# prototypefund/your-voice-TTS

Measured on AMD Instinct MI355X. Metric: mel-frames/sec + RTF, Tacotron2 + 60-iter Griffin-Lim, LJSpeech, higher is better.
Workload: dtype f32; 1 GPU; configs[1]: Tacotron2 single sentence, HIP decoder loop + HIP Griffin-Lim 60 iters; sentences_per_gpu=1, L=100, gl_iters=60, model_config=config_tacotron2.json + forward_attn_mask (synthesize.py:86), parallelism=single GPU

## Files before the change

include/tts_hip.h:

```cpp
#ifndef TTS_HIP_H
#define TTS_HIP_H

#include <stdint.h>

#ifdef __cplusplus
extern "C" {
#endif

typedef int tts_status;
#define TTS_OK 0
#define TTS_ERR_INVALID 1
#define TTS_ERR_HIP 2
#define TTS_ERR_UNSUPPORTED 3
#define TTS_ERR_NOMEM 4

typedef struct tts_encoder tts_encoder;
typedef struct tts_decoder tts_decoder;
typedef struct tts_postnet tts_postnet;
typedef struct tts_gl tts_gl;
typedef struct tts_tacotron tts_tacotron;

typedef struct tts_tensor {
    const char* key;
    const float* data;
    int64_t numel;
} tts_tensor;

tts_status tts_encoder_create(const tts_tensor* tensors, int n_tensors, int max_batch, int max_len,
                              void* stream, tts_encoder** out);
void tts_encoder_destroy(tts_encoder* e);
tts_status tts_encoder_run(tts_encoder* e, const int32_t* ids, const int32_t* lens, int B, int Lmax,
                           float* out, void* stream);
tts_status tts_encoder_run_state(tts_encoder* e, const int32_t* ids, const int32_t* lens, int B, int Lmax,
                                 const float* state_in, float* state_out, float* out, void* stream);

tts_status tts_encoder_add_speakers(tts_encoder* e, float* enc, const int32_t* lens, const int32_t* speaker_ids, int B,
                                    int Lmax, void* stream);

tts_status tts_encoder_last_path(tts_encoder* e, int* resident);

typedef struct tts_decoder_config {
    int r;
    int attn_norm;
    int forward_attn;
    int trans_agent;
    int forward_attn_mask;
    int location_attn;
    int windowing;
    int max_batch;
    int max_len;
    int max_steps;
} tts_decoder_config;

tts_status tts_decoder_create(const tts_decoder_config* cfg, const tts_tensor* tensors, int n_tensors,
                              void* stream, tts_decoder** out);
void tts_decoder_destroy(tts_decoder* d);

tts_status tts_decoder_run(tts_decoder* d, const float* enc, const int32_t* lens, int B, int Lmax,
                           int max_steps, int steps_cap, float* mel, float* stop, float* align,
                           int32_t* n_steps, void* stream);

tts_status tts_decoder_run_continue(tts_decoder* d, const float* enc, const int32_t* lens, int B, int Lmax,
                                    int max_steps, int steps_cap, float* mel, float* stop, float* align,
                                    int32_t* n_steps, void* stream);

tts_status tts_decoder_run_teacher(tts_decoder* d, const float* enc, const int32_t* lens, int B, int Lmax,
                                   const float* memories, int64_t mem_ldb, int steps, float* mel, float* stop,
                                   float* align, void* stream);

tts_status tts_decoder_last_timing(tts_decoder* d, float* loop_ms, int* steps_run);

tts_status tts_decoder_last_path(tts_decoder* d, int* resident);
// ... 56 lines not shown
                           const int32_t* orig_sr, int target_sr, int B, double* dst, int64_t dst_pitch,
                           int32_t* n_out, void* stream);

tts_status tts_gl_set_mel_basis(tts_gl* g, const double* mel_basis);
tts_status tts_gl_melspectrogram(tts_gl* g, const double* wav, const int32_t* N, int B, int64_t Nmax, float* mel,
                                 int Fmax, void* stream);

tts_status tts_gl_analyze(tts_gl* g, const double* wav, const int32_t* N, int B, int64_t Nmax, float* linear,
                          float* mel, int Fmax, void* stream);

tts_status tts_gl_linear_to_mel(tts_gl* g, const float* linear, const int32_t* F, int B, int Fmax, float* mel,
                                void* stream);

tts_status tts_gl_last_timing(tts_gl* g, float* loop_ms, int* launches);

#define TTS_GL_PATH_UNFUSED 0
#define TTS_GL_PATH_FUSED 1
#define TTS_GL_PATH_PERSISTENT 2
tts_status tts_gl_last_path(tts_gl* g, int* path);

#define TTS_GL_KERNELS 2
tts_status tts_gl_profile(tts_gl* g, int reps, float* kernel_ms, int n_kernels);

typedef struct tts_synth tts_synth;
tts_status tts_synth_create(tts_encoder* e, tts_decoder* d, tts_postnet* p, tts_gl* g, int r, int n_mel, int hop,
                            tts_synth** out);
void tts_synth_destroy(tts_synth* s);
tts_status tts_synth_run(tts_synth* s, const int32_t* ids, const int32_t* lens, int B, int Lmax, int max_steps,
                         int gl_iters, uint64_t seed, double* wav, int64_t wav_cap, int32_t* frames, void* stream);
tts_status tts_synth_run_speakers(tts_synth* s, const int32_t* ids, const int32_t* lens, const int32_t* speaker_ids,
                                  int B, int Lmax, int max_steps, int gl_iters, uint64_t seed, double* wav,
                                  int64_t wav_cap, int32_t* frames, void* stream);
tts_status tts_synth_sync(tts_synth* s);

#define TTS_TACOTRON_MEMORY_SIZE_MAX 16
typedef struct tts_tacotron_config {
    int r;
    int memory_size;
    int attn_norm;
    int forward_attn, trans_agent, forward_attn_mask, location_attn, windowing;
    int gst;
    int num_speakers;
    int max_batch;
    int max_len;
    int max_steps;
} tts_tacotron_config;

tts_status tts_tacotron_create(const tts_tacotron_config* cfg, const tts_tensor* tensors, int n_tensors,
                               void* stream, tts_tacotron** out);
void tts_tacotron_destroy(tts_tacotron* t);

tts_status tts_tacotron_encode(tts_tacotron* t, const int32_t* ids, const int32_t* lens, int B, int Lmax,
                               const int32_t* speaker_ids, const float* style_mel, int style_frames, float* out,
                               void* stream);

tts_status tts_tacotron_decode(tts_tacotron* t, const float* enc, const int32_t* lens, int B, int Lmax,
                               int max_steps, int steps_cap, float* mel, float* stop, float* align,
                               int32_t* n_steps, void* stream);

tts_status tts_tacotron_decode_teacher(tts_tacotron* t, const float* enc, const int32_t* lens, int B, int Lmax,
                                       const float* memories, int64_t mem_ldb, int steps, float* mel,
                                       float* stop, float* align, void* stream);

tts_status tts_tacotron_postnet(tts_tacotron* t, const float* mel, const int32_t* T, int B, int Tmax,
                                float* linear, void* stream);

// ... 70 lines not shown
```

your-voice-tts_amd/_native.py:

```python
from __future__ import annotations

import ctypes
import os
import threading

_HERE = os.path.dirname(os.path.abspath(__file__))
LIB_PATH = os.environ.get("TTS_HIP_LIB", os.path.join(_HERE, "libtts_hip.so"))

TTS_GL_FROM_MEL = 0
TTS_GL_FROM_LINEAR = 1
TTS_LOSS_L1 = 0
TTS_LOSS_MSE = 1
TTS_LOSS_BCE = 2
TTS_OPTIM_CHUNK = 8192
GL_PATHS = {0: "unfused", 1: "fused", 2: "persistent"}
DECODER_STEP_KERNELS = ("prenet2", "att_lstm", "query", "attention", "dec_lstm", "mel_fused")
GL_KERNELS = ("gl_iter", "gl_ola")
TACOTRON_STEP_KERNELS = ("prenet2", "att_gru", "query", "attention", "proj", "dec_gru1", "dec_gru2", "mel",
                         "pre1_stop")

EXPORTS = (
    "tts_encoder_create", "tts_encoder_destroy", "tts_encoder_run", "tts_encoder_run_state", "tts_encoder_last_path",
    "tts_encoder_add_speakers", "tts_synth_run_speakers",
    "tts_decoder_create", "tts_decoder_destroy", "tts_decoder_run", "tts_decoder_run_continue", "tts_decoder_run_teacher",
    "tts_decoder_last_timing", "tts_decoder_last_path", "tts_decoder_resident_limits", "tts_decoder_resident_phases", "tts_decoder_resident_trace",
    "tts_decoder_profile",
    "tts_postnet_create", "tts_postnet_destroy", "tts_postnet_run", "tts_postnet_last_path",
    "tts_gl_create", "tts_gl_destroy", "tts_gl_run", "tts_gl_last_timing", "tts_gl_last_path", "tts_gl_profile",
    "tts_gl_set_mel_basis", "tts_gl_melspectrogram", "tts_gl_set_phase_state", "tts_gl_get_phase_state",
    "tts_gl_draw_phases", "tts_gl_save_pcm16", "tts_gl_analyze", "tts_gl_linear_to_mel",
    "tts_gl_trim_silence", "tts_gl_find_endpoint", "tts_gl_take_segments",
    "tts_gl_set_resample_filter", "tts_gl_resample",
    "tts_synth_create", "tts_synth_destroy", "tts_synth_run", "tts_synth_sync",
    "tts_tacotron_create", "tts_tacotron_destroy", "tts_tacotron_encode", "tts_tacotron_decode",
    "tts_tacotron_decode_teacher",
    "tts_tacotron_postnet", "tts_tacotron_last_timing", "tts_tacotron_last_path", "tts_tacotron_resident_phases",
    "tts_tacotron_profile",
    "tts_loss_create", "tts_loss_destroy", "tts_loss_masked", "tts_loss_bce_logits", "tts_loss_backward",
    "tts_optim_create", "tts_optim_destroy", "tts_optim_set_tensors", "tts_optim_grad_norm", "tts_optim_clip",
    "tts_optim_decay", "tts_optim_adam", "tts_optim_step",
    "tts_last_error", "tts_version",
)


class TensorView(ctypes.Structure):
    _fields_ = [("key", ctypes.c_char_p), ("data", ctypes.c_void_p), ("numel", ctypes.c_int64)]


class DecoderConfig(ctypes.Structure):
    _fields_ = [(n, ctypes.c_int) for n in (
        "r", "attn_norm", "forward_attn", "trans_agent", "forward_attn_mask", "location_attn",
        "windowing", "max_batch", "max_len", "max_steps")]


class TacotronConfig(ctypes.Structure):
    _fields_ = [(n, ctypes.c_int) for n in (
# ... 14 lines not shown
                ("signal_norm", ctypes.c_int), ("symmetric_norm", ctypes.c_int), ("clip_norm", ctypes.c_int)]


_lib = None
_lock = threading.Lock()
P = ctypes.c_void_p
I32P = ctypes.POINTER(ctypes.c_int32)


def _declare(lib):
    vp = ctypes.c_void_p
    lib.tts_encoder_create.argtypes = [ctypes.POINTER(TensorView), ctypes.c_int, ctypes.c_int, ctypes.c_int, vp,
                                       ctypes.POINTER(vp)]
    lib.tts_encoder_destroy.argtypes = [vp]
    lib.tts_encoder_destroy.restype = None
    lib.tts_encoder_run.argtypes = [vp, vp, I32P, ctypes.c_int, ctypes.c_int, vp, vp]
    lib.tts_encoder_add_speakers.argtypes = [vp, vp, I32P, I32P, ctypes.c_int, ctypes.c_int, vp]
    lib.tts_decoder_create.argtypes = [ctypes.POINTER(DecoderConfig), ctypes.POINTER(TensorView), ctypes.c_int, vp,
                                       ctypes.POINTER(vp)]
    lib.tts_decoder_destroy.argtypes = [vp]
    lib.tts_decoder_destroy.restype = None
    lib.tts_decoder_run.argtypes = [vp, vp, I32P, ctypes.c_int, ctypes.c_int, ctypes.c_int, ctypes.c_int, vp, vp, vp,
                                    I32P, vp]
    lib.tts_encoder_run_state.argtypes = [vp, vp, I32P, ctypes.c_int, ctypes.c_int, vp, vp, vp, vp]
    lib.tts_decoder_run_continue.argtypes = lib.tts_decoder_run.argtypes
    lib.tts_decoder_run_teacher.argtypes = [vp, vp, I32P, ctypes.c_int, ctypes.c_int, vp, ctypes.c_int64, ctypes.c_int,
                                            vp, vp, vp, vp]
    lib.tts_decoder_last_timing.argtypes = [vp, ctypes.POINTER(ctypes.c_float), ctypes.POINTER(ctypes.c_int)]
    lib.tts_decoder_last_path.argtypes = [vp, ctypes.POINTER(ctypes.c_int)]
    lib.tts_decoder_resident_limits.argtypes = [vp, ctypes.POINTER(ctypes.c_int), ctypes.POINTER(ctypes.c_int)]
    lib.tts_encoder_last_path.argtypes = [vp, ctypes.POINTER(ctypes.c_int)]
    lib.tts_gl_last_path.argtypes = [vp, ctypes.POINTER(ctypes.c_int)]
    lib.tts_synth_sync.argtypes = [vp]
    lib.tts_decoder_resident_phases.argtypes = [vp, ctypes.POINTER(ctypes.c_float), ctypes.c_int]
    lib.tts_decoder_resident_trace.argtypes = [vp, ctypes.POINTER(ctypes.c_longlong), ctypes.c_int64]
    lib.tts_postnet_create.argtypes = [ctypes.POINTER(TensorView), ctypes.c_int, ctypes.c_int, vp, ctypes.POINTER(vp)]
    lib.tts_postnet_destroy.argtypes = [vp]
    lib.tts_postnet_destroy.restype = None
    lib.tts_postnet_run.argtypes = [vp, vp, I32P, ctypes.c_int, ctypes.c_int, vp, vp]
    lib.tts_postnet_last_path.argtypes = [vp, ctypes.POINTER(ctypes.c_int), ctypes.c_int]
    lib.tts_gl_create.argtypes = [ctypes.POINTER(AudioConfig), vp, vp, ctypes.POINTER(vp)]
    lib.tts_gl_destroy.argtypes = [vp]
    lib.tts_gl_destroy.restype = None
    lib.tts_gl_run.argtypes = [vp, ctypes.c_int, vp, I32P, ctypes.c_int, ctypes.c_int, vp, ctypes.c_uint64,
                               ctypes.c_int, vp, vp]
    lib.tts_gl_set_mel_basis.argtypes = [vp, vp]
    lib.tts_gl_melspectrogram.argtypes = [vp, vp, I32P, ctypes.c_int, ctypes.c_int64, vp, ctypes.c_int, vp]
    lib.tts_gl_analyze.argtypes = [vp, vp, I32P, ctypes.c_int, ctypes.c_int64, vp, vp, ctypes.c_int, vp]
    lib.tts_gl_linear_to_mel.argtypes = [vp, vp, I32P, ctypes.c_int, ctypes.c_int, vp, vp]
    lib.tts_gl_last_timing.argtypes = [vp, ctypes.POINTER(ctypes.c_float), ctypes.POINTER(ctypes.c_int)]
    U32P = ctypes.POINTER(ctypes.c_uint32)
    lib.tts_gl_set_phase_state.argtypes = [vp, U32P, ctypes.c_int]
    lib.tts_gl_get_phase_state.argtypes = [vp, U32P, ctypes.POINTER(ctypes.c_int)]
    lib.tts_gl_draw_phases.argtypes = [vp, I32P, ctypes.c_int, ctypes.c_int, vp, vp]
    lib.tts_gl_save_pcm16.argtypes = [vp, vp, ctypes.c_int64, ctypes.POINTER(ctypes.c_int64), ctypes.c_int, ctypes.c_int,
                                      ctypes.c_double, vp, vp]
    lib.tts_gl_trim_silence.argtypes = [vp, vp, ctypes.c_int64, I32P, ctypes.c_int, ctypes.c_int, ctypes.c_int,
                                        ctypes.c_int, ctypes.c_double, I32P, I32P, vp]
    lib.tts_gl_find_endpoint.argtypes = [vp, vp, ctypes.c_int64, I32P, ctypes.c_int, ctypes.c_int, ctypes.c_int,
                                         ctypes.c_double, I32P, vp]
    lib.tts_gl_take_segments.argtypes = [vp, vp, ctypes.c_int64, I32P, I32P, ctypes.c_int, vp, ctypes.c_int64, vp]
    lib.tts_gl_set_resample_filter.argtypes = [vp, vp, ctypes.c_int, ctypes.c_int]
    lib.tts_gl_resample.argtypes = [vp, vp, ctypes.c_int64, I32P, I32P, ctypes.c_int, ctypes.c_int, vp, ctypes.c_int64,
                                    I32P, vp]
    lib.tts_synth_create.argtypes = [vp, vp, vp, vp, ctypes.c_int, ctypes.c_int, ctypes.c_int, ctypes.POINTER(vp)]
    lib.tts_synth_destroy.argtypes = [vp]
# ... 16 lines not shown
                                                ctypes.c_int, vp, vp, vp, vp]
    lib.tts_tacotron_postnet.argtypes = [vp, vp, I32P, ctypes.c_int, ctypes.c_int, vp, vp]
    lib.tts_tacotron_last_timing.argtypes = [vp, ctypes.POINTER(ctypes.c_float), ctypes.POINTER(ctypes.c_int)]
    lib.tts_tacotron_last_path.argtypes = [vp, ctypes.POINTER(ctypes.c_int)]
    lib.tts_tacotron_resident_phases.argtypes = [vp, FP, ctypes.c_int]
    lib.tts_tacotron_profile.argtypes = [vp, ctypes.c_int, FP, ctypes.c_int]
    DP, I64P = ctypes.POINTER(ctypes.c_double), ctypes.POINTER(ctypes.c_int64)
    lib.tts_loss_create.argtypes = [ctypes.POINTER(vp)]
    lib.tts_loss_destroy.argtypes = [vp]
    lib.tts_loss_destroy.restype = None
    lib.tts_loss_masked.argtypes = [vp, ctypes.c_int, vp, ctypes.c_int64, vp, ctypes.c_int64, I32P, ctypes.c_int,
                                    ctypes.c_int, ctypes.c_int, vp, vp, DP, I64P, DP, vp]
    lib.tts_loss_bce_logits.argtypes = [vp, vp, vp, ctypes.c_int64, vp, vp, DP, DP, vp]
    lib.tts_loss_backward.argtypes = [ctypes.c_int, vp, ctypes.c_int64, vp, ctypes.c_int64, vp, ctypes.c_int,
                                      ctypes.c_int64, ctypes.c_int64, vp, vp, ctypes.c_int64, vp]
    OT, D = ctypes.POINTER(OptimTensor), ctypes.c_double
    lib.tts_optim_create.argtypes = [ctypes.POINTER(vp)]
    lib.tts_optim_destroy.argtypes = [vp]
    lib.tts_optim_destroy.restype = None
    lib.tts_optim_set_tensors.argtypes = [vp, I64P, ctypes.c_int, vp]
    lib.tts_optim_grad_norm.argtypes = [vp, OT, ctypes.c_int, D, vp, vp, DP, DP, vp]
    lib.tts_optim_clip.argtypes = lib.tts_optim_grad_norm.argtypes
    lib.tts_optim_decay.argtypes = [vp, OT, ctypes.c_int, D, D, vp]
    lib.tts_optim_adam.argtypes = [vp, OT, ctypes.c_int, D, D, D, D, vp]
    lib.tts_optim_step.argtypes = [vp, OT, ctypes.c_int, D, D, D, D, D, D, vp, vp, vp]
    lib.tts_last_error.restype = ctypes.c_char_p
    lib.tts_version.restype = ctypes.c_char_p
    for name in EXPORTS:
        fn = getattr(lib, name)
        if name.endswith(("_create", "_run", "_timing", "_profile", "_encode", "_decode", "_postnet", "_state",
                          "_continue", "_basis", "_melspectrogram", "_path", "_sync", "_phases", "_teacher",
                          "_phase_state", "_pcm16", "_limits", "_analyze", "_to_mel", "_silence", "_endpoint",
                          "_segments", "_masked", "_logits", "_filter", "_resample", "_tensors", "_grad_norm",
                          "_clip", "_decay", "_adam", "_step", "_backward")):
            fn.restype = ctypes.c_int


def load_library(path: str = LIB_PATH):
    global _lib
    with _lock:
        if _lib is None:
            import torch
            if not os.path.exists(path):
                raise RuntimeError(f"libtts_hip.so not found at {path}: build it with "
                                   f"`make -C your-voice-tts_amd/csrc` (no CPU fallback exists)")
            lib = ctypes.CDLL(path)
            _declare(lib)
            _lib = lib
    return _lib


def lib():
    import torch
    if not torch.cuda.is_available():
        raise RuntimeError("no GPU visible: the MI355X synthesis path has no CPU fallback")
    return load_library()


def check(status: int, what: str):
    if status != 0:
        msg = load_library().tts_last_error().decode(errors="replace")
        if "attention norm" in msg:
            raise RuntimeError("Unknown value for attention norm type")
        raise RuntimeError(f"{what} failed (status {status}): {msg}")


def stream_handle(stream=None):
# ... 23 lines not shown
```

your-voice-tts_amd/csrc/encoder_api.hip:

```cpp
#include <algorithm>
#include <map>
#include <string>

#include "conv1d.h"
#include "encoder_resident.h"
#include "host_util.h"
#include "resident.h"
#include "sgemm.h"

using namespace tts;

namespace {
constexpr int EDIM = 512;
constexpr int EH = 256;
constexpr int EG = 4 * EH;
}

struct tts_encoder {
    int num_chars = 0, Bcap = 0, Lcap = 0;
    hipStream_t stream = nullptr;
    hipEvent_t ev_in = nullptr, ev_out = nullptr;
    DeviceAllocs dev;
    float* emb = nullptr;
    float* spk = nullptr;
    int nspk = 0;
    float *Wc[3] = {}, *sc[3] = {}, *sh[3] = {};
    float *Wp = nullptr, *bp = nullptr;
    float *Wcf[3] = {}, *Wpf = nullptr;
    float* Wcf16[3] = {};
    float* Whh = nullptr;
    int *ids = nullptr, *T = nullptr;
    float *act0 = nullptr, *act1 = nullptr, *xi = nullptr, *h = nullptr, *c = nullptr, *out = nullptr;
    float* part = nullptr;
    std::map<std::pair<int, int>, hipGraphExec_t> graphs;
    bool resident = false;
    float4* rw = nullptr;
    unsigned long long* rgran = nullptr;
    long long rtmo = 0;
    unsigned rsalt = 0;
    bool rgran_clear = false;
    unsigned rsalt_pending = 0;
    bool pending_batch = false;
    int* host_status = nullptr;
    bool pipeline = false;
    bool status_pending = false;
    bool defer_status = false;
    bool lens_staged = false;
    bool skip_resident_once = false;
    int res_timeouts = 0;
    std::map<int, hipGraphExec_t> rgraphs;
    float* whh_raw = nullptr;
    unsigned long long* bgran = nullptr;
    unsigned bsalt = 0;
    bool bgran_clear = false;
    std::map<std::pair<int, int>, hipGraphExec_t> bgraphs;
    int last_resident = 0;
};

namespace {

__global__ void zero_rows_past_len_kernel(float* out, int Lmax, const int* T) {
    const int t = blockIdx.x, b = blockIdx.y;
    if (t < T[b]) return;
    reinterpret_cast<float4*>(out + ((size_t)b * Lmax + t) * EDIM)[threadIdx.x] = float4{0.f, 0.f, 0.f, 0.f};
}

tts_status enqueue_encoder(tts_encoder* e, int B, int Lmax, int frames, hipStream_t s, bool resident = false) {
    if (!(resident && B == 1)) {
        hipLaunchKernelGGL(zero_rows_past_len_kernel, dim3(Lmax, B), dim3(EDIM / 4), 0, s, e->out, Lmax, e->T);
        TTS_HIP(hipGetLastError());
    }
    float* bufs[2] = {e->act0, e->act1};
    for (int l = 0; l < 3; ++l) {
        ConvArgs a{};
        a.in = l == 0 ? nullptr : bufs[(l - 1) & 1];
        a.ids = l == 0 ? e->ids : nullptr;
        a.table = e->emb;
        a.out = bufs[l & 1];
        a.W = e->Wc[l];
        a.Wf = e->Wcf[l];
        a.Wf16 = e->Wcf16[l];
        a.wf_tap = conv_frag_tap_ok(EDIM) ? 1 : 0;
// ... 54 lines not shown
        E.enc_out = e->out;
        TTS_HIP(sgemm_launch(a, ROLE_ENC_LSTM, s));
    }
    return TTS_OK;
}

tts_status enqueue_encoder_resident(tts_encoder* e, int Lmax, bool zero_state, hipStream_t s, bool* launched) {
    const int64_t hs = (int64_t)e->Bcap * EH;
    bool wrapped = false;
    e->rsalt = res_next_salt(e->rsalt, &wrapped);
    if (wrapped || !e->rgran_clear)
        TTS_HIP(hipMemsetAsync(e->rgran, 0, sizeof(unsigned long long) * encoder_resident_granules(), s));
    e->rgran_clear = true;
    EncResArgs a{};
    a.w = e->rw;
    static const int enc_first_sleep = env_int("TTS_ENC_FIRST_SLEEP", 2);
    a.first_sleep = enc_first_sleep;
    a.xi = e->xi;
    a.L = Lmax;
    a.hdir = hs;
    a.h0 = zero_state ? nullptr : e->h + 2 * hs;
    a.c0 = zero_state ? nullptr : e->c;
    a.h_fin = e->h + (int64_t)((Lmax - 1) & 1) * 2 * hs;
    a.c_fin = e->c;
    a.out = e->out;
    a.gran = e->rgran;
    a.status = reinterpret_cast<int*>(e->rgran + encoder_resident_granules() - 2);
    a.tmo = e->rtmo;
    a.salt = e->rsalt;
    TTS_HIP(launch_encoder_resident(a, s, launched));
    return TTS_OK;
}

}

extern "C" {

void tts_encoder_destroy(tts_encoder* e) {
    if (!e) return;
    if (e->stream) (void)hipStreamSynchronize(e->stream);
    for (auto& kv : e->graphs) (void)hipGraphExecDestroy(kv.second);
    for (auto& kv : e->rgraphs) (void)hipGraphExecDestroy(kv.second);
    for (auto& kv : e->bgraphs) (void)hipGraphExecDestroy(kv.second);
    if (e->host_status) (void)hipHostFree(e->host_status);
    e->dev.free_all();
    for (hipEvent_t ev : {e->ev_in, e->ev_out})
        if (ev) (void)hipEventDestroy(ev);
    if (e->stream) (void)hipStreamDestroy(e->stream);
    delete e;
}

tts_status tts_encoder_create(const tts_tensor* tensors, int n_tensors, int max_batch, int max_len, void* stream,
                              tts_encoder** out) {
    TTS_CHECK(tensors && out, TTS_ERR_INVALID, "null argument");
    TTS_CHECK(max_batch >= 1 && max_batch <= 64, TTS_ERR_UNSUPPORTED, "max_batch must be in [1, 64]");
    TTS_CHECK(max_len >= 1 && max_len <= 4096, TTS_ERR_UNSUPPORTED, "max_len must be in [1, 4096]");
    const WeightMap weights(tensors, n_tensors);
    const auto& wm = weights.m;
    auto get = [&](const std::string& k, int64_t numel) { return weights.get(k, numel); };
    auto* e = new tts_encoder();
    hipStream_t s = static_cast<hipStream_t>(stream);
    auto fail = [&](tts_status code) { tts_encoder_destroy(e); return code; };
    tts_status st = TTS_OK;
#define CK(x)                    \
    do {                         \
        st = (x);                \
        if (st) return fail(st); \
    } while (0)
#define HK(x)                                                                    \
// ... 151 lines not shown
                tts_status st = enqueue_encoder(e, 1, Lmax, Lmax, s, true);
                hipError_t ee = hipStreamEndCapture(s, &g);
                if (st) return st;
                TTS_HIP(ee);
                hipGraphExec_t exec = nullptr;
                TTS_HIP(hipGraphInstantiate(&exec, g, nullptr, nullptr, 0));
                TTS_HIP(hipGraphDestroy(g));
                rit = e->rgraphs.emplace(Lmax, exec).first;
            }
            TTS_HIP(hipGraphLaunch(rit->second, s));
        }
        bool launched = false;
        {
            tts_status st = enqueue_encoder_resident(e, Lmax, !state_in, s, &launched);
            if (st) return st;
        }
        if (!launched) {
            e->resident = false;
            if (!state_in) {
                if (tts_status st = init_state()) return st;
            }
        } else {
            e->last_resident = 1;
            e->rsalt_pending = e->rsalt;
            e->pending_batch = false;
            if (!(e->pipeline && e->defer_status))
                TTS_HIP(hipMemcpyAsync(e->host_status, e->rgran + encoder_resident_granules() - 2, sizeof(int),
                                       hipMemcpyDeviceToHost, s));
            if (e->pipeline) {
                e->status_pending = true;
                goto done;
            }
            TTS_HIP(hipStreamSynchronize(s));
            e->host_status[0] = res_status_code(e->host_status[0], e->rsalt);
            if (e->host_status[0] == ENC_RES_STATUS_PLACEMENT) {
                e->resident = false;
                if (tts_status st = init_state()) return st;
            } else if (e->host_status[0] != 0) {
                ++e->res_timeouts;
                if (tts_status st = init_state()) return st;
            } else {
                goto done;
            }
        }
    }
    static const bool batch_off = env_is("TTS_ENC_BATCH_RESIDENT", '0');
    if (e->resident && e->bgran && !skip_resident && B >= 2 && !state_in && !batch_off) {
        auto key = std::make_pair(B, Lmax);
        auto bit = e->bgraphs.find(key);
        if (bit == e->bgraphs.end()) {
            hipGraph_t g = nullptr;
            TTS_HIP(hipStreamBeginCapture(s, hipStreamCaptureModeThreadLocal));
            tts_status st = enqueue_encoder(e, B, Lmax, B * Lmax, s, true);
            hipError_t ee = hipStreamEndCapture(s, &g);
            if (st) return st;
            TTS_HIP(ee);
            hipGraphExec_t exec = nullptr;
            TTS_HIP(hipGraphInstantiate(&exec, g, nullptr, nullptr, 0));
            TTS_HIP(hipGraphDestroy(g));
            bit = e->bgraphs.emplace(key, exec).first;
        }
        TTS_HIP(hipGraphLaunch(bit->second, s));
        bool wrapped = false;
        e->bsalt = res_next_salt(e->bsalt, &wrapped);
        if (wrapped || !e->bgran_clear)
            TTS_HIP(hipMemsetAsync(e->bgran, 0, sizeof(unsigned long long) * encoder_resident_batch_granules(), s));
        e->bgran_clear = true;
        EncResBatchArgs ba{};
        ba.whh = e->whh_raw;
        ba.xi = e->xi;
        ba.lens = e->T;
        ba.B = B;
        ba.Tmax = Lmax;
        ba.out = e->out;
        ba.hdir = (int64_t)hs;
        ba.h_fin = e->h;
// ... 52 lines not shown
            }
        }
    }
    if (s != cs) {
        TTS_HIP(hipEventRecord(e->ev_out, s));
        TTS_HIP(hipStreamWaitEvent(cs, e->ev_out, 0));
    }
    return TTS_OK;
}

}

namespace tts {
void encoder_set_pipeline(tts_encoder* e, bool on) {
    e->pipeline = on;
    if (!on) e->defer_status = e->lens_staged = false;
}
void encoder_set_lens_staged(tts_encoder* e, bool staged) { e->lens_staged = staged; }
int32_t* encoder_ids_buffer(tts_encoder* e, int B, int Lmax) {
    return (size_t)B * Lmax <= (size_t)e->Bcap * e->Lcap ? e->ids : nullptr;
}
float* encoder_out_buffer(tts_encoder* e) { return e->out; }
const int* encoder_lens_buffer(tts_encoder* e) { return e->T; }
void encoder_status_words(tts_encoder* e, const int** dev, int** host) {
    *dev = e->rgran ? reinterpret_cast<const int*>(e->rgran + encoder_resident_granules() - 2) : nullptr;
    *host = e->host_status;
}
void encoder_set_defer_status(tts_encoder* e, bool defer) { e->defer_status = defer; }

tts_status encoder_pending_status(tts_encoder* e, int* placement_failed) {
    *placement_failed = 0;
    if (!e->status_pending) return TTS_OK;
    e->status_pending = false;
    e->host_status[0] = res_status_code(e->host_status[0], e->rsalt_pending);
    if (e->host_status[0] == ENC_RES_STATUS_PLACEMENT) {
        if (e->pending_batch) e->bgran = nullptr;
        else e->resident = false;
        *placement_failed = 1;
        return TTS_OK;
    }
    if (e->host_status[0] != 0) {
        ++e->res_timeouts;
        e->skip_resident_once = true;
        *placement_failed = 1;
    }
    return TTS_OK;
}
}

namespace {
struct SpeakerAdd {
    int spk[64];
    int len[64];
};
__global__ void speaker_add_kernel(float* enc, int Lmax, const float* table, const SpeakerAdd a) {
    const int t = blockIdx.x, b = blockIdx.y;
    if (t >= a.len[b]) return;
    float4* row = reinterpret_cast<float4*>(enc + ((size_t)b * Lmax + t) * EDIM) + threadIdx.x;
    const float4 v = reinterpret_cast<const float4*>(table + (size_t)a.spk[b] * EDIM)[threadIdx.x];
    const float4 x = *row;
    *row = float4{x.x + v.x, x.y + v.y, x.z + v.z, x.w + v.w};
}
}

namespace tts {
tts_status encoder_add_speakers(tts_encoder* e, float* enc, const int32_t* lens, const int32_t* speaker_ids, int B,
                                int Lmax, hipStream_t s) {
    TTS_CHECK(e && enc && lens && speaker_ids, TTS_ERR_INVALID, "null argument");
    TTS_CHECK(e->spk, TTS_ERR_INVALID, "speaker embeddings need speaker_embedding.weight at tts_encoder_create");
    TTS_CHECK(B >= 1 && B <= 64 && B <= e->Bcap && Lmax >= 1, TTS_ERR_INVALID, "bad batch for speaker embeddings");
// ... 46 lines not shown
```

your-voice-tts_amd/csrc/synth_api.hip:

```cpp
#include <hip/hip_runtime.h>

#include <algorithm>
#include <cstdio>
#include <vector>

#include "common.h"
#include "host_util.h"

struct tts_synth {
    tts_encoder* e = nullptr;
    tts_decoder* d = nullptr;
    tts_postnet* p = nullptr;
    tts_gl* g = nullptr;
    int r = 1, nmel = 80, hop = 0;
    int32_t* ids = nullptr;
    float *enc = nullptr, *mel = nullptr, *stop = nullptr;
    float *post[2] = {nullptr, nullptr}, *spec[2] = {nullptr, nullptr};
    size_t ids_n = 0, enc_n = 0, mel_n = 0, stop_n = 0, spec_n = 0;
    std::vector<int32_t> steps;
    hipStream_t stream = nullptr, gl_stream = nullptr;
    hipEvent_t ev_in = nullptr, ev_post = nullptr, ev_out = nullptr;
    int32_t* pin[2] = {nullptr, nullptr};
    size_t pin_n[2] = {0, 0};
    unsigned calls = 0;
    int* fspec = nullptr;
    hipStream_t last_cs = nullptr;
};

namespace {
template <typename T>
tts_status grow(T** p, size_t& have, size_t need) {
    if (need <= have) return TTS_OK;
    if (*p) TTS_HIP(hipFree(*p));
    *p = nullptr;
    TTS_HIP(hipMalloc(reinterpret_cast<void**>(p), need * sizeof(T)));
    have = need;
    return TTS_OK;
}

struct PipelineScope {
    tts_synth* s;
    explicit PipelineScope(tts_synth* x) : s(x) { set(true); }
    ~PipelineScope() { set(false); }
    void set(bool on) {
        tts::encoder_set_pipeline(s->e, on);
        tts::decoder_set_pipeline(s->d, on);
        tts::gl_set_pipeline(s->g, on);
    }
};

tts_status synth_stages(tts_synth* s, int32_t* h_ids, int32_t* h_lens, const int32_t* spk, int32_t* h_frames, int B,
                        int Lmax, int max_steps, int gl_iters, uint64_t seed, double* wav, int64_t wav_cap,
                        int32_t* frames, void* stream);
tts_status synth_run(tts_synth* s, const int32_t* ids, const int32_t* lens, const int32_t* spk, int B, int Lmax,
                     int max_steps, int gl_iters, uint64_t seed, double* wav, int64_t wav_cap, int32_t* frames,
                     void* stream);
}

extern "C" {

tts_status tts_synth_create(tts_encoder* e, tts_decoder* d, tts_postnet* p, tts_gl* g, int r, int n_mel, int hop,
                            tts_synth** out) {
    TTS_CHECK(e && d && p && g && out, TTS_ERR_INVALID, "null handle");
    TTS_CHECK(r >= 1 && n_mel >= 1 && hop >= 1, TTS_ERR_INVALID, "bad r / n_mel / hop");
    tts_synth* s = new tts_synth;
    s->e = e;
    s->d = d;
    s->p = p;
    s->g = g;
    s->r = r;
    s->nmel = n_mel;
    s->hop = hop;
    int prio_lo = 0, prio_hi = 0;
    if (tts::env_is("TTS_STREAM_PRIO", '1'))
        if (hipDeviceGetStreamPriorityRange(&prio_lo, &prio_hi) != hipSuccess) prio_lo = prio_hi = 0;
    if (hipStreamCreateWithPriority(&s->stream, hipStreamNonBlocking, prio_hi) != hipSuccess ||
        hipStreamCreateWithPriority(&s->gl_stream, hipStreamNonBlocking, prio_lo) != hipSuccess ||
        hipEventCreateWithFlags(&s->ev_in, hipEventDisableTiming) != hipSuccess ||
        hipEventCreateWithFlags(&s->ev_post, hipEventDisableTiming) != hipSuccess ||
        hipEventCreateWithFlags(&s->ev_out, hipEventDisableTiming) != hipSuccess ||
        hipMalloc(&s->fspec, 4 * sizeof(int)) != hipSuccess) {
        tts_synth_destroy(s);
        tts::set_error("tts_synth_create: stream / event creation failed");
        return TTS_ERR_HIP;
    }
    *out = s;
    return TTS_OK;
}

void tts_synth_destroy(tts_synth* s) {
    if (!s) return;
    for (hipStream_t q : {s->stream, s->gl_stream})
        if (q) (void)hipStreamSynchronize(q);
    if (s->last_cs) (void)hipDeviceSynchronize();
    if (tts::gl_collect(s->g) != TTS_OK)
        std::fprintf(stderr, "tts_synth_destroy: the last run failed: %s\n", tts_last_error());
    for (void* q : {(void*)s->ids, (void*)s->enc, (void*)s->mel, (void*)s->stop, (void*)s->post[0],
                    (void*)s->post[1], (void*)s->spec[0], (void*)s->spec[1], (void*)s->fspec})
        if (q) (void)hipFree(q);
    for (int32_t* q : s->pin)
        if (q) (void)hipHostFree(q);
    for (hipEvent_t ev : {s->ev_in, s->ev_post, s->ev_out})
        if (ev) (void)hipEventDestroy(ev);
    for (hipStream_t q : {s->stream, s->gl_stream})
        if (q) (void)hipStreamDestroy(q);
    delete s;
}

tts_status tts_synth_run(tts_synth* s, const int32_t* ids, const int32_t* lens, int B, int Lmax, int max_steps,
                         int gl_iters, uint64_t seed, double* wav, int64_t wav_cap, int32_t* frames, void* stream) {
    return synth_run(s, ids, lens, nullptr, B, Lmax, max_steps, gl_iters, seed, wav, wav_cap, frames, stream);
}

tts_status tts_synth_run_speakers(tts_synth* s, const int32_t* ids, const int32_t* lens, const int32_t* speaker_ids,
                                  int B, int Lmax, int max_steps, int gl_iters, uint64_t seed, double* wav,
                                  int64_t wav_cap, int32_t* frames, void* stream) {
    TTS_CHECK(speaker_ids, TTS_ERR_INVALID, "null speaker_ids");
    return synth_run(s, ids, lens, speaker_ids, B, Lmax, max_steps, gl_iters, seed, wav, wav_cap, frames, stream);
}
}

namespace {
tts_status synth_run(tts_synth* s, const int32_t* ids, const int32_t* lens, const int32_t* spk, int B, int Lmax,
                     int max_steps, int gl_iters, uint64_t seed, double* wav, int64_t wav_cap, int32_t* frames,
                     void* stream) {
    TTS_CHECK(s && ids && lens && wav && frames && B >= 1 && Lmax >= 2 && max_steps >= 1 && gl_iters >= 0,
              TTS_ERR_INVALID, "bad synth arguments");
    hipStream_t ss = s->stream;
    const int cap = max_steps + 21;
    const size_t T = (size_t)cap * s->r;
    tts_status st;
    hipStream_t cs = static_cast<hipStream_t>(stream);
    const bool regrow = (size_t)B * Lmax > s->ids_n || (size_t)B * Lmax * 512 > s->enc_n ||
                        (size_t)B * T * s->nmel > s->mel_n || (size_t)B * cap > s->stop_n;
    const int par = s->calls & 1;
    const size_t pin_need = (size_t)B * Lmax + 2 * (size_t)B;
    if (regrow || pin_need > s->pin_n[par]) {
        TTS_HIP(hipStreamSynchronize(ss));
        TTS_HIP(hipStreamSynchronize(s->gl_stream));
        TTS_HIP(hipStreamSynchronize(cs));
    }
    if ((st = grow(&s->ids, s->ids_n, (size_t)B * Lmax))) return st;
    if ((st = grow(&s->enc, s->enc_n, (size_t)B * Lmax * 512))) return st;
    if ((st = grow(&s->mel, s->mel_n, (size_t)B * T * s->nmel))) return st;
    if ((st = grow(&s->stop, s->stop_n, (size_t)B * cap))) return st;
    if (!s->post[0] || s->spec_n < s->mel_n) {
        for (int k = 0; k < 2; ++k) {
            if (s->post[k]) TTS_HIP(hipFree(s->post[k]));
            if (s->spec[k]) TTS_HIP(hipFree(s->spec[k]));
            s->post[k] = s->spec[k] = nullptr;
        }
        for (int k = 0; k < 2; ++k) {
            TTS_HIP(hipMalloc(&s->post[k], s->mel_n * sizeof(float)));
            TTS_HIP(hipMalloc(&s->spec[k], s->mel_n * sizeof(float)));
        }
        s->spec_n = s->mel_n;
    }
    if (pin_need > s->pin_n[par]) {
        if (s->pin[par]) TTS_HIP(hipHostFree(s->pin[par]));
        s->pin[par] = nullptr;
        TTS_HIP(hipHostMalloc(reinterpret_cast<void**>(&s->pin[par]), pin_need * sizeof(int32_t)));
        s->pin_n[par] = pin_need;
    }
    int32_t* h_ids = s->pin[par];
    int32_t* h_lens = h_ids + (size_t)B * Lmax;
    int32_t* h_frames = h_lens + B;
    std::copy(ids, ids + (size_t)B * Lmax, h_ids);
    std::copy(lens, lens + B, h_lens);
    st = synth_stages(s, h_ids, h_lens, spk, h_frames, B, Lmax, max_steps, gl_iters, seed, wav, wav_cap, frames, stream);
    if (st) {
        (void)hipStreamSynchronize(s->stream);
        (void)hipStreamSynchronize(s->gl_stream);
        (void)hipStreamSynchronize(cs);
        return st;
    }
    ++s->calls;
    return TTS_OK;
}
}

extern "C" {
tts_status tts_synth_sync(tts_synth* s) {
    TTS_CHECK(s, TTS_ERR_INVALID, "null handle");
    TTS_HIP(hipStreamSynchronize(s->stream));
    TTS_HIP(hipStreamSynchronize(s->gl_stream));
    if (s->last_cs) TTS_HIP(hipStreamSynchronize(s->last_cs));
    return tts::gl_collect(s->g);
}

}

namespace {
tts_status synth_stages(tts_synth* s, int32_t* h_ids, int32_t* h_lens, const int32_t* spk, int32_t* h_frames, int B,
                        int Lmax, int max_steps, int gl_iters, uint64_t seed, double* wav, int64_t wav_cap,
                        int32_t* frames, void* stream) {
    hipStream_t cs = static_cast<hipStream_t>(stream);
    static const bool own_stream = tts::env_is("TTS_SYNTH_OWN_STREAM", '1');
    hipStream_t ss = B == 1 && !own_stream ? cs : s->stream;
    s->last_cs = ss == cs ? cs : nullptr;
    const int cap = max_steps + 21;
    const size_t T = (size_t)cap * s->r;
    tts_status st;
    const int par = s->calls & 1;
    PipelineScope scope(s);
    int32_t* ids_dev = tts::encoder_ids_buffer(s->e, B, Lmax);
    if (!ids_dev) ids_dev = s->ids;
    float* const enc = tts::encoder_out_buffer(s->e);
    if (B == 1 && Lmax <= tts::STAGE_IDS_MAX && ids_dev != s->ids) {
        tts::StageIds sa;
        sa.ids = ids_dev;
        sa.lens = const_cast<int*>(tts::encoder_lens_buffer(s->e));
        sa.n = Lmax;
        sa.len = h_lens[0];
        std::copy(h_ids, h_ids + Lmax, sa.v);
        TTS_HIP(tts::stage_ids(sa, ss));
        tts::encoder_set_lens_staged(s->e, true);
    } else {
        TTS_HIP(hipMemcpyAsync(ids_dev, h_ids, sizeof(int32_t) * (size_t)B * Lmax, hipMemcpyHostToDevice, ss));
        tts::encoder_set_lens_staged(s->e, false);
    }
    s->steps.assign(B, 0);
    const float* hist = nullptr;
    int64_t sent_floats = 0;
    const int* n_dev = nullptr;
    tts::decoder_histories(s->d, &hist, &sent_floats, &n_dev);
    float* const post = s->post[par];
    const int Ts = (int)std::min<size_t>(256, T);
    const int Tp = (int)std::min<size_t>(1024, T);
    static const bool no_spec = tts::env_is("TTS_NO_SPEC_GL", '1');
    const bool spec_gl = B == 1 && s->r == 1 && !no_spec && wav_cap >= (int64_t)s->hop * (Ts - 1) &&
                         tts::gl_persistent_path(s->g, 1, Ts, Ts, gl_iters);
    struct Hook {
        tts_synth* s;
        const float* hist;
        int mel_tmax;
        const int* n_dev;
        float* post;
        int T, Tp;
        tts_status st;
        bool spec_gl;
        int Ts;
        uint64_t seed;
        int iters;
        double* wav;
        hipStream_t cs;
        bool gl_done;
    } hook{s, hist, (int)(sent_floats / s->nmel), n_dev, post, (int)T, Tp, TTS_OK, spec_gl, Ts, seed, gl_iters, wav, cs, false};
    auto hook_fn = [](void* c, hipStream_t q) {
        Hook* h = static_cast<Hook*>(c);
        const int32_t Tcap[1] = {h->Tp};
        h->st = tts::postnet_run_dev(h->s->p, h->hist, h->mel_tmax, h->n_dev, h->s->r, Tcap, 1, h->T, h->post, q);
        if (h->st || !h->spec_gl) return;
        const hipError_t idle = q == h->cs ? hipSuccess : hipStreamQuery(h->cs);
        if (idle != hipSuccess && idle != hipErrorNotReady) {
            h->st = TTS_ERR_HIP;
            tts::set_error("tts_synth_run: caller stream query failed");
            return;
        }
        if (idle == hipErrorNotReady &&
            (hipEventRecord(h->s->ev_in, h->cs) != hipSuccess || hipStreamWaitEvent(q, h->s->ev_in, 0) != hipSuccess)) {
            h->st = TTS_ERR_HIP;
            tts::set_error("tts_synth_run: event hand-off failed");
            return;
        }
        const int32_t Fb[1] = {h->Ts};
        h->st = tts::gl_run_dev(h->s->g, TTS_GL_FROM_MEL, h->post, Fb, h->s->fspec, 1, h->Ts, nullptr, h->seed, h->iters,
                                h->wav, q, true);
        h->gl_done = h->st == TTS_OK;
    };
    if (B == 1) {
        const int* est = nullptr;
        int* ehost = nullptr;
        tts::encoder_status_words(s->e, &est, &ehost);
        tts::encoder_set_defer_status(s->e, est != nullptr);
        tts::decoder_set_pipeline_io(s->d, tts::encoder_lens_buffer(s->e), est, ehost, spec_gl ? s->fspec : nullptr, Ts);
    }
    static const bool no_hook = tts::env_is("TTS_NO_HOOK", '1');
    tts::decoder_set_post_hook(s->d, B == 1 && !no_hook ? +hook_fn : nullptr, &hook);
    for (int attempt = 0;; ++attempt) {
        if ((st = tts_encoder_run(s->e, ids_dev, h_lens, B, Lmax, enc, ss))) return st;
        if (spk && (st = tts::encoder_add_speakers(s->e, enc, h_lens, spk, B, Lmax, ss))) return st;
        st = tts_decoder_run(s->d, enc, h_lens, B, Lmax, max_steps, cap, s->mel, s->stop, nullptr, s->steps.data(), ss);
        if (!st) st = hook.st;
        if (st) {
            tts::decoder_set_post_hook(s->d, nullptr, nullptr);
            return st;
        }
        int rerun = 0;
        if ((st = tts::encoder_pending_status(s->e, &rerun))) return st;
        if (!rerun) break;
        TTS_CHECK(attempt == 0, TTS_ERR_HIP, "encoder rerun failed (internal error)");
    }
    int Fmax = 0;
    for (int b = 0; b < B; ++b) {
        h_frames[b] = s->steps[b] * s->r;
        Fmax = std::max(Fmax, (int)h_frames[b]);
    }
    TTS_CHECK(Fmax >= 2, TTS_ERR_INVALID, "a sentence decoded to fewer than 2 frames");
    TTS_CHECK(wav_cap >= (int64_t)B * s->hop * (Fmax - 1), TTS_ERR_INVALID, "wav buffer too small");
    std::copy(h_frames, h_frames + B, frames);
    const bool post_done = tts::decoder_hook_ran(s->d) && Fmax <= Tp;
    const bool gl_done = post_done && hook.gl_done && Fmax <= Ts;
    tts::decoder_set_post_hook(s->d, nullptr, nullptr);
    if (!post_done) {
        if ((st = tts::postnet_run_dev(s->p, hist, (int)(sent_floats / s->nmel), n_dev, s->r, h_frames, B, (int)T, post, ss)))
            return st;
    }
    const float* spec = post;
    if (B > 1) {
        const size_t row = (size_t)s->nmel * sizeof(float);
        TTS_HIP(hipMemcpy2DAsync(s->spec[par], Fmax * row, post, T * row, Fmax * row, B, hipMemcpyDeviceToDevice, ss));
        spec = s->spec[par];
    }
    int frames_total = 0;
// ... 28 lines not shown
```

your-voice-tts_amd/tacotron2.py:

```python
from __future__ import annotations

import ctypes
from collections import OrderedDict

import numpy as np
import torch

from . import _native, weights


def _speaker_array(speaker_ids, B):
    spk = np.asarray(torch.as_tensor(speaker_ids).view(-1).cpu().numpy(), dtype=np.int32)
    if spk.size == 1 and B > 1:
        spk = np.repeat(spk, B)
    if spk.size != B:
        raise ValueError(f"speaker_ids has {spk.size} entries for a batch of {B}")
    return np.ascontiguousarray(spk)


class _DecoderAttrs:

    def __init__(self, r):
        self.max_decoder_steps = 1000
        self.r = r
# ... 289 lines not shown
            _native.check(lib.tts_synth_create(self._native[3], hdec, hpost, hgl, self.n_frames_per_step, 80,
                                               ap.hop_length, ctypes.byref(hs)), "tts_synth_create")
            self._synth = (hs, key, ap)
        hs = self._synth[0]
        max_steps = int(self.decoder.max_decoder_steps)
        ids = np.zeros((B, Lmax), np.int32)
        for b, x in enumerate(ids_list):
            ids[b, :lens[b]] = np.asarray(x, dtype=np.int32)
        cap = self.native_wav_capacity(ap, B)
        if out is not None:
            if out.dtype != torch.float64 or not out.is_cuda or not out.is_contiguous() or out.numel() < cap:
                raise ValueError(f"out must be a contiguous CUDA float64 buffer of >= {cap} elements")
            wav_buf = out
        else:
            if self._wav_buf is None or self._wav_buf.numel() < cap:
                self._wav_buf = torch.empty(cap, dtype=torch.float64, device=self.device)
            wav_buf = self._wav_buf
        frames = (ctypes.c_int32 * B)()
        iters = ap.griffin_lim_iters if iters is None else iters
        if speaker_ids is None:
            _native.check(lib.tts_synth_run(hs, ids.ctypes.data_as(_native.I32P), _native.i32_array(lens), B, Lmax,
                                            max_steps, int(iters), int(seed), ctypes.c_void_p(wav_buf.data_ptr()),
                                            cap, frames, _native.stream_handle()), "tts_synth_run")
        else:
            spk = _speaker_array(speaker_ids, B)
            _native.check(lib.tts_synth_run_speakers(hs, ids.ctypes.data_as(_native.I32P), _native.i32_array(lens),
                                                     _native.i32_array(spk), B, Lmax, max_steps, int(iters), int(seed),
                                                     ctypes.c_void_p(wav_buf.data_ptr()), cap, frames,
                                                     _native.stream_handle()), "tts_synth_run_speakers")
        frames = [int(f) for f in frames]
        if sync:
            _native.check(lib.tts_synth_sync(hs), "tts_synth_sync")
        self.last_timing = self._path_timing(lib, hdec)
        self.last_lengths = frames
        n = ap.hop_length * (max(frames) - 1)
        return wav_buf.view(-1)[:B * n].view(B, n), frames

    def native_wav_capacity(self, ap, B=1):
        return B * ap.hop_length * ((int(self.decoder.max_decoder_steps) + 21) * self.n_frames_per_step - 1)

    def resident_limits(self, Lmax=1):
        lib, hdec, _ = self._handles(max(int(Lmax), 1), 1)
        mb, ml = ctypes.c_int(), ctypes.c_int()
        _native.check(lib.tts_decoder_resident_limits(hdec, ctypes.byref(mb), ctypes.byref(ml)),
                      "tts_decoder_resident_limits")
        return mb.value, ml.value

    def synth_sync(self):
        if self._synth is not None:
            _native.check(_native.lib().tts_synth_sync(self._synth[0]), "tts_synth_sync")

    def _path_timing(self, lib, hdec):
        ms, ns, res, enc = ctypes.c_float(), ctypes.c_int(), ctypes.c_int(), ctypes.c_int()
        lib.tts_decoder_last_timing(hdec, ctypes.byref(ms), ctypes.byref(ns))
        lib.tts_decoder_last_path(hdec, ctypes.byref(res))
        lib.tts_encoder_last_path(self._native[3], ctypes.byref(enc))
        return dict(decoder_loop_ms=ms.value, decoder_steps_run=ns.value, resident=bool(res.value),
                    resident_kind=int(res.value), encoder_resident=bool(enc.value), encoder_path=int(enc.value))

    RESIDENT_PHASES = ("att_early_wait_pre1", "prenet2_row", "wait_prenet2", "att_lstm_prenet", "att_cell_gather",
                       "query_dec_early", "wait_query", "energies_max", "weights_ctx_publish", "dec_lstm_hatt",
                       "wait_ctx", "dec_lstm_ctx", "dec_cell_gather", "fused_rows", "cand_energies", "weights_ctx")

    def profile_resident_phases(self):
        lib, hdec, _ = self._handles(1, 1)
        n = 2 * len(self.RESIDENT_PHASES)
        us = (ctypes.c_float * n)()
        _native.check(lib.tts_decoder_resident_phases(hdec, us, n), "tts_decoder_resident_phases")
        k = len(self.RESIDENT_PHASES)
        return {"cu0": dict(zip(self.RESIDENT_PHASES, [float(v) for v in us[:k]])),
                "attention_cu": dict(zip(self.RESIDENT_PHASES, [float(v) for v in us[k:]]))}

    def profile_resident_trace(self):
        lib, hdec, _ = self._handles(1, 1)
        n = 256 * 64 * 16
        buf = (ctypes.c_longlong * n)()
        _native.check(lib.tts_decoder_resident_trace(hdec, buf, n), "tts_decoder_resident_trace")
        return np.frombuffer(buf, dtype=np.int64).reshape(256, 64, 16).copy()

    def profile_step_kernels(self, reps=50):
        lib, hdec, _ = self._handles(1, 1)
        n = len(_native.DECODER_STEP_KERNELS)
        ms = (ctypes.c_float * n)()
        _native.check(lib.tts_decoder_profile(hdec, int(reps), ms, n), "tts_decoder_profile")
        return dict(zip(_native.DECODER_STEP_KERNELS, [float(v) for v in ms]))

    @torch.no_grad()
    def inference_truncated(self, text, speaker_ids=None):
        _native.lib()
        text = torch.as_tensor(text)
        if text.dim() == 1:
# ... 24 lines not shown
```

Before: 103,400 mel-frames/s.

## Run encoder on side stream when caller stream is busy to overlap prior work

```diff
diff --git a/include/tts_hip.h b/include/tts_hip.h
--- a/include/tts_hip.h
+++ b/include/tts_hip.h
@@ -38,6 +38,11 @@
                                     int Lmax, void* stream);
 
 tts_status tts_encoder_last_path(tts_encoder* e, int* resident);
+tts_status tts_encoder_counters(tts_encoder* e, int* placement_failures, int* timeouts);
+#define TTS_ENC_RUN_OK 0
+#define TTS_ENC_RUN_PLACEMENT 1
+#define TTS_ENC_RUN_TIMEOUT 2
+tts_status tts_encoder_status_rule(int status_word, unsigned salt, int* fails_in_row, int* resident, int* outcome);
 
 typedef struct tts_decoder_config {
     int r;
@@ -160,6 +165,7 @@
                                   int B, int Lmax, int max_steps, int gl_iters, uint64_t seed, double* wav,
                                   int64_t wav_cap, int32_t* frames, void* stream);
 tts_status tts_synth_sync(tts_synth* s);
+tts_status tts_synth_state(tts_synth* s, int* last_front, int* in_flight);
 
 #define TTS_TACOTRON_MEMORY_SIZE_MAX 16
 typedef struct tts_tacotron_config {
diff --git a/your-voice-tts_amd/_native.py b/your-voice-tts_amd/_native.py
--- a/your-voice-tts_amd/_native.py
+++ b/your-voice-tts_amd/_native.py
@@ -22,6 +22,7 @@
 EXPORTS = (
     "tts_encoder_create", "tts_encoder_destroy", "tts_encoder_run", "tts_encoder_run_state", "tts_encoder_last_path",
     "tts_encoder_add_speakers", "tts_synth_run_speakers",
+    "tts_encoder_counters", "tts_encoder_status_rule", "tts_synth_state",
     "tts_decoder_create", "tts_decoder_destroy", "tts_decoder_run", "tts_decoder_run_continue", "tts_decoder_run_teacher",
     "tts_decoder_last_timing", "tts_decoder_last_path", "tts_decoder_resident_limits", "tts_decoder_resident_phases", "tts_decoder_resident_trace",
     "tts_decoder_profile",
@@ -102,6 +103,10 @@
     lib.tts_encoder_last_path.argtypes = [vp, ctypes.POINTER(ctypes.c_int)]
     lib.tts_gl_last_path.argtypes = [vp, ctypes.POINTER(ctypes.c_int)]
     lib.tts_synth_sync.argtypes = [vp]
+    IP = ctypes.POINTER(ctypes.c_int)
+    lib.tts_encoder_counters.argtypes = [vp, IP, IP]
+    lib.tts_encoder_status_rule.argtypes = [ctypes.c_int, ctypes.c_uint, IP, IP, IP]
+    lib.tts_synth_state.argtypes = [vp, IP, IP]
     lib.tts_decoder_resident_phases.argtypes = [vp, ctypes.POINTER(ctypes.c_float), ctypes.c_int]
     lib.tts_decoder_resident_trace.argtypes = [vp, ctypes.POINTER(ctypes.c_longlong), ctypes.c_int64]
     lib.tts_postnet_create.argtypes = [ctypes.POINTER(TensorView), ctypes.c_int, ctypes.c_int, vp, ctypes.POINTER(vp)]
@@ -184,7 +189,7 @@
                           "_continue", "_basis", "_melspectrogram", "_path", "_sync", "_phases", "_teacher",
                           "_phase_state", "_pcm16", "_limits", "_analyze", "_to_mel", "_silence", "_endpoint",
                           "_segments", "_masked", "_logits", "_filter", "_resample", "_tensors", "_grad_norm",
-                          "_clip", "_decay", "_adam", "_step", "_backward")):
+                          "_clip", "_decay", "_adam", "_step", "_backward", "_counters", "_rule")):
             fn.restype = ctypes.c_int
 
 
diff --git a/your-voice-tts_amd/csrc/encoder_api.hip b/your-voice-tts_amd/csrc/encoder_api.hip
--- a/your-voice-tts_amd/csrc/encoder_api.hip
+++ b/your-voice-tts_amd/csrc/encoder_api.hip
@@ -48,6 +48,8 @@
     bool lens_staged = false;
     bool skip_resident_once = false;
     int res_timeouts = 0;
+    int res_place_fails = 0;
+    int res_placements = 0;
     std::map<int, hipGraphExec_t> rgraphs;
     float* whh_raw = nullptr;
     unsigned long long* bgran = nullptr;
@@ -168,9 +170,41 @@
     return TTS_OK;
 }
 
+int resident_outcome(tts_encoder* e, unsigned salt) {
+    int outcome = TTS_ENC_RUN_OK, resident = e->resident ? 1 : 0;
+    (void)tts_encoder_status_rule(e->host_status[0], salt, &e->res_place_fails, &resident, &outcome);
+    e->host_status[0] = res_status_code(e->host_status[0], salt);
+    e->resident = resident != 0;
+    if (outcome == TTS_ENC_RUN_PLACEMENT) ++e->res_placements;
+    if (outcome == TTS_ENC_RUN_TIMEOUT) ++e->res_timeouts;
+    return outcome;
+}
+
 }
 
 extern "C" {
+
+tts_status tts_encoder_status_rule(int status_word, unsigned salt, int* fails_in_row, int* resident, int* outcome) {
+    TTS_CHECK(fails_in_row && resident && outcome, TTS_ERR_INVALID, "null argument");
+    const int code = res_status_code(status_word, salt);
+    if (code == ENC_RES_STATUS_PLACEMENT) {
+        if (++*fails_in_row >= RES_PLACEMENT_RETRIES) *resident = 0;
+        *outcome = TTS_ENC_RUN_PLACEMENT;
+    } else if (code != 0) {
+        *outcome = TTS_ENC_RUN_TIMEOUT;
+    } else {
+        *fails_in_row = 0;
+        *outcome = TTS_ENC_RUN_OK;
+    }
+    return TTS_OK;
+}
+
+tts_status tts_encoder_counters(tts_encoder* e, int* placement_failures, int* timeouts) {
+    TTS_CHECK(e && placement_failures && timeouts, TTS_ERR_INVALID, "null argument");
+    *placement_failures = e->res_placements;
+    *timeouts = e->res_timeouts;
+    return TTS_OK;
+}
 
 void tts_encoder_destroy(tts_encoder* e) {
     if (!e) return;
@@ -388,16 +422,8 @@
                 goto done;
             }
             TTS_HIP(hipStreamSynchronize(s));
-            e->host_status[0] = res_status_code(e->host_status[0], e->rsalt);
-            if (e->host_status[0] == ENC_RES_STATUS_PLACEMENT) {
-                e->resident = false;
-                if (tts_status st = init_state()) return st;
-            } else if (e->host_status[0] != 0) {
-                ++e->res_timeouts;
-                if (tts_status st = init_state()) return st;
-            } else {
-                goto done;
-            }
+            if (resident_outcome(e, e->rsalt) == TTS_ENC_RUN_OK) goto done;
+            if (tts_status st = init_state()) return st;
         }
     }
     static const bool batch_off = env_is("TTS_ENC_BATCH_RESIDENT", '0');
@@ -516,10 +542,16 @@
     *placement_failed = 0;
     if (!e->status_pending) return TTS_OK;
     e->status_pending = false;
+    if (!e->pending_batch) {
+        if (resident_outcome(e, e->rsalt_pending) != TTS_ENC_RUN_OK) {
+            e->skip_resident_once = true;
+            *placement_failed = 1;
+        }
+        return TTS_OK;
+    }
     e->host_status[0] = res_status_code(e->host_status[0], e->rsalt_pending);
     if (e->host_status[0] == ENC_RES_STATUS_PLACEMENT) {
-        if (e->pending_batch) e->bgran = nullptr;
-        else e->resident = false;
+        e->bgran = nullptr;
         *placement_failed = 1;
         return TTS_OK;
     }
diff --git a/your-voice-tts_amd/csrc/synth_api.hip b/your-voice-tts_amd/csrc/synth_api.hip
--- a/your-voice-tts_amd/csrc/synth_api.hip
+++ b/your-voice-tts_amd/csrc/synth_api.hip
@@ -20,6 +20,8 @@
     std::vector<int32_t> steps;
     hipStream_t stream = nullptr, gl_stream = nullptr;
     hipEvent_t ev_in = nullptr, ev_post = nullptr, ev_out = nullptr;
+    hipEvent_t ev_front = nullptr;
+    bool last_front = false;
     int32_t* pin[2] = {nullptr, nullptr};
     size_t pin_n[2] = {0, 0};
     unsigned calls = 0;
@@ -51,7 +53,7 @@
 
 tts_status synth_stages(tts_synth* s, int32_t* h_ids, int32_t* h_lens, const int32_t* spk, int32_t* h_frames, int B,
                         int Lmax, int max_steps, int gl_iters, uint64_t seed, double* wav, int64_t wav_cap,
-                        int32_t* frames, void* stream);
+                        int32_t* frames, void* stream, bool cs_busy);
 tts_status synth_run(tts_synth* s, const int32_t* ids, const int32_t* lens, const int32_t* spk, int B, int Lmax,
                      int max_steps, int gl_iters, uint64_t seed, double* wav, int64_t wav_cap, int32_t* frames,
                      void* stream);
@@ -79,6 +81,7 @@
         hipEventCreateWithFlags(&s->ev_in, hipEventDisableTiming) != hipSuccess ||
         hipEventCreateWithFlags(&s->ev_post, hipEventDisableTiming) != hipSuccess ||
         hipEventCreateWithFlags(&s->ev_out, hipEventDisableTiming) != hipSuccess ||
+        hipEventCreateWithFlags(&s->ev_front, hipEventDisableTiming) != hipSuccess ||
         hipMalloc(&s->fspec, 4 * sizeof(int)) != hipSuccess) {
         tts_synth_destroy(s);
         tts::set_error("tts_synth_create: stream / event creation failed");
@@ -100,7 +103,7 @@
         if (q) (void)hipFree(q);
     for (int32_t* q : s->pin)
         if (q) (void)hipHostFree(q);
-    for (hipEvent_t ev : {s->ev_in, s->ev_post, s->ev_out})
+    for (hipEvent_t ev : {s->ev_in, s->ev_post, s->ev_out, s->ev_front})
         if (ev) (void)hipEventDestroy(ev);
     for (hipStream_t q : {s->stream, s->gl_stream})
         if (q) (void)hipStreamDestroy(q);
@@ -131,6 +134,8 @@
     const size_t T = (size_t)cap * s->r;
     tts_status st;
     hipStream_t cs = static_cast<hipStream_t>(stream);
+    const bool cs_busy = hipStreamQuery(cs) == hipErrorNotReady;
+    (void)hipGetLastError();
     const bool regrow = (size_t)B * Lmax > s->ids_n || (size_t)B * Lmax * 512 > s->enc_n ||
                         (size_t)B * T * s->nmel > s->mel_n || (size_t)B * cap > s->stop_n;
     const int par = s->calls & 1;
@@ -167,7 +172,8 @@
     int32_t* h_frames = h_lens + B;
     std::copy(ids, ids + (size_t)B * Lmax, h_ids);
     std::copy(lens, lens + B, h_lens);
-    st = synth_stages(s, h_ids, h_lens, spk, h_frames, B, Lmax, max_steps, gl_iters, seed, wav, wav_cap, frames, stream);
+    st = synth_stages(s, h_ids, h_lens, spk, h_frames, B, Lmax, max_steps, gl_iters, seed, wav, wav_cap, frames, stream,
+                      cs_busy);
     if (st) {
         (void)hipStreamSynchronize(s->stream);
         (void)hipStreamSynchronize(s->gl_stream);
@@ -188,16 +194,33 @@
     return tts::gl_collect(s->g);
 }
 
+tts_status tts_synth_state(tts_synth* s, int* last_front, int* in_flight) {
+    TTS_CHECK(s && last_front, TTS_ERR_INVALID, "null argument");
+    *last_front = s->last_front ? 1 : 0;
+    if (!in_flight) return TTS_OK;
+    *in_flight = 0;
+    for (hipStream_t q : {s->stream, s->gl_stream, s->last_cs}) {
+        const hipError_t e = hipStreamQuery(q);
+        (void)hipGetLastError();
+        if (e == hipErrorNotReady) *in_flight = 1;
+        else TTS_HIP(e);
+    }
+    return TTS_OK;
+}
+
 }
 
 namespace {
 tts_status synth_stages(tts_synth* s, int32_t* h_ids, int32_t* h_lens, const int32_t* spk, int32_t* h_frames, int B,
                         int Lmax, int max_steps, int gl_iters, uint64_t seed, double* wav, int64_t wav_cap,
-                        int32_t* frames, void* stream) {
+                        int32_t* frames, void* stream, bool cs_busy) {
     hipStream_t cs = static_cast<hipStream_t>(stream);
     static const bool own_stream = tts::env_is("TTS_SYNTH_OWN_STREAM", '1');
     hipStream_t ss = B == 1 && !own_stream ? cs : s->stream;
     s->last_cs = ss == cs ? cs : nullptr;
+    const bool front = ss == cs && cs_busy && !tts::env_is("TTS_SYNTH_FRONT", '0');
+    s->last_front = front;
+    hipStream_t es = front ? s->stream : ss;
     const int cap = max_steps + 21;
     const size_t T = (size_t)cap * s->r;
     tts_status st;
@@ -213,10 +236,10 @@
         sa.n = Lmax;
         sa.len = h_lens[0];
         std::copy(h_ids, h_ids + Lmax, sa.v);
-        TTS_HIP(tts::stage_ids(sa, ss));
+        TTS_HIP(tts::stage_ids(sa, es));
         tts::encoder_set_lens_staged(s->e, true);
     } else {
-        TTS_HIP(hipMemcpyAsync(ids_dev, h_ids, sizeof(int32_t) * (size_t)B * Lmax, hipMemcpyHostToDevice, ss));
+        TTS_HIP(hipMemcpyAsync(ids_dev, h_ids, sizeof(int32_t) * (size_t)B * Lmax, hipMemcpyHostToDevice, es));
         tts::encoder_set_lens_staged(s->e, false);
     }
     s->steps.assign(B, 0);
@@ -278,8 +301,13 @@
     static const bool no_hook = tts::env_is("TTS_NO_HOOK", '1');
     tts::decoder_set_post_hook(s->d, B == 1 && !no_hook ? +hook_fn : nullptr, &hook);
     for (int attempt = 0;; ++attempt) {
-        if ((st = tts_encoder_run(s->e, ids_dev, h_lens, B, Lmax, enc, ss))) return st;
-        if (spk && (st = tts::encoder_add_speakers(s->e, enc, h_lens, spk, B, Lmax, ss))) return st;
+        if (attempt == 1) es = ss;
+        if ((st = tts_encoder_run(s->e, ids_dev, h_lens, B, Lmax, enc, es))) return st;
+        if (spk && (st = tts::encoder_add_speakers(s->e, enc, h_lens, spk, B, Lmax, es))) return st;
+        if (es != ss) {
+            TTS_HIP(hipEventRecord(s->ev_front, es));
+            TTS_HIP(hipStreamWaitEvent(ss, s->ev_front, 0));
+        }
         st = tts_decoder_run(s->d, enc, h_lens, B, Lmax, max_steps, cap, s->mel, s->stop, nullptr, s->steps.data(), ss);
         if (!st) st = hook.st;
         if (st) {
diff --git a/your-voice-tts_amd/tacotron2.py b/your-voice-tts_amd/tacotron2.py
--- a/your-voice-tts_amd/tacotron2.py
+++ b/your-voice-tts_amd/tacotron2.py
@@ -345,6 +345,9 @@
         if sync:
             _native.check(lib.tts_synth_sync(hs), "tts_synth_sync")
         self.last_timing = self._path_timing(lib, hdec)
+        front = ctypes.c_int()
+        _native.check(lib.tts_synth_state(hs, ctypes.byref(front), None), "tts_synth_state")
+        self.last_timing["encoder_front"] = bool(front.value)
         self.last_lengths = frames
         n = ap.hop_length * (max(frames) - 1)
         return wav_buf.view(-1)[:B * n].view(B, n), frames
@@ -368,8 +371,11 @@
         lib.tts_decoder_last_timing(hdec, ctypes.byref(ms), ctypes.byref(ns))
         lib.tts_decoder_last_path(hdec, ctypes.byref(res))
         lib.tts_encoder_last_path(self._native[3], ctypes.byref(enc))
+        npl, ntm = ctypes.c_int(), ctypes.c_int()
+        lib.tts_encoder_counters(self._native[3], ctypes.byref(npl), ctypes.byref(ntm))
         return dict(decoder_loop_ms=ms.value, decoder_steps_run=ns.value, resident=bool(res.value),
-                    resident_kind=int(res.value), encoder_resident=bool(enc.value), encoder_path=int(enc.value))
+                    resident_kind=int(res.value), encoder_resident=bool(enc.value), encoder_path=int(enc.value),
+                    encoder_placement_failures=npl.value, encoder_timeouts=ntm.value)
 
     RESIDENT_PHASES = ("att_early_wait_pre1", "prenet2_row", "wait_prenet2", "att_lstm_prenet", "att_cell_gather",
                        "query_dec_early", "wait_query", "energies_max", "weights_ctx_publish", "dec_lstm_hatt",
```

Result: faster. 108,900 mel-frames/s (median of 6 runs) (+5.3%).
